# CederGroupHub/sparse-lm

Measured on AMD Instinct MI355X. Metric: fits/sec over 50-alpha Lasso path at n=100k p=5k, higher is better.
Workload: dtype f64

## Files before the change

### sparse-lm_amd/csrc/ws_kernels.hpp

```cpp
#pragma once
#include <type_traits>
#include <hip/hip_runtime.h>
#include <stdint.h>

#include "tail_kernels.hpp"
#include "newton_kernels.hpp"

namespace slm {

constexpr int WS_KCAP = 512;
constexpr int WS_KLDS = 112;
constexpr int WS_TILES = WS_KCAP / 16;
constexpr int WS_THREADS = 1024;
constexpr int WS_INNER_MAX = 400;
constexpr int WS_BB_ITERS = 14;
constexpr double WS_BB_MAX_STEP = 20.0;
constexpr double WS_INNER_TOL = 0.05;
constexpr int WS_MAX_REPEATS = 6;
constexpr int WS_NEWTON_AFTER = 16;
constexpr int WS_NEWTON_MAX = 256;
constexpr int WS_AFTER_DIRECT = 40;
constexpr double WS_NEWTON_RQ = 0.05;
constexpr int WS_NEWTON_REFUSALS = 4;
constexpr double WS_NEWTON_ENTER = 0.3;
constexpr int WS_NEWTON_RESOLVE = 5;
static_assert(NT_MAXT * NT_B == WS_KCAP, "the direct solve covers a full working set");

struct WsCtl {
  int32_t request;
  int32_t building;
  int32_t valid;
  int32_t K;
  int32_t Kreal;
  int32_t k_new;
  int32_t builds;
  int32_t appends;
  int32_t max_builds;
  int32_t disabled;
  int32_t misses;
  int32_t refined;
  int32_t counter;
  int32_t stale;
  int32_t overflows;
  int32_t sweep_new;
  int32_t sweep_miss;
  int32_t staged;
  int32_t inner_iters;
  int32_t hard;
  int32_t hard_next;
  int32_t newton_steps;
  int32_t newton_fails;
  int32_t newton_nopd;
  int32_t newton_trial[4];
  int32_t newton_ref[4];
  int32_t newton_factors;
  int32_t newton_unknowns;
  unsigned long long nt_ticks[SLM_MAX_LANES][6];
  int32_t nt_factors[SLM_MAX_LANES];
  unsigned long long solve_ticks[5];
  int32_t want_full[SLM_MAX_LANES];
  int32_t iters_hist[32];
  unsigned long long lane_ticks[SLM_MAX_LANES];
  int32_t last_point[SLM_MAX_LANES];
  int32_t repeats[SLM_MAX_LANES];
  int32_t last_cols[SLM_MAX_LANES];
  double Lw[SLM_MAX_LANES];
  int32_t carried;
  int32_t outgrown;
  int32_t served[SLM_MAX_LANES];
  int32_t hard_lane[SLM_MAX_LANES];
};

struct WsArgs {
  WsCtl* ws;
  int32_t* idx;
  int32_t* pos;
  int32_t* gs;
  int32_t* gl;
  double* score;
  double* XW;
  double* part;
  double* Gm;
  double* nt;
  double* Gx;
  const double* X;
  const double* XT;
  int64_t n, ld;
  const double* rw;
  int64_t rw_stride;
  double inv_n[SLM_MAX_LANES];
  int32_t set_of[SLM_MAX_LANES];
  int32_t set_lane[SLM_MAX_LANES];
  int32_t n_sets;
  int32_t nblk;
  const int32_t* owner;
  double theta;
  int32_t lookahead;
  int32_t append_max;
  int32_t k_init;
  int32_t bb_steps;
  int32_t one_solver;
  int32_t miss_factor;
  int32_t miss_div;
  double fill;
  int32_t power_iters;
  int32_t hard_call;
  int32_t keep_full;
};

constexpr int WS_HEAD_WORDS = 24;
static_assert(offsetof(WsCtl, hard_next) / 4 < WS_HEAD_WORDS, "the words the pass kernels decide on");
#define WS_HEAD(hd, field) ((hd)[offsetof(WsCtl, field) / 4])
__device__ __forceinline__ void ws_head_load(const WsCtl* ws, const int* gdone, int32_t* hd) {
  const int tid = threadIdx.x;
  if (tid < WS_HEAD_WORDS) hd[tid] = reinterpret_cast<const int32_t*>(ws)[tid];
  else if (tid == WS_HEAD_WORDS) hd[tid] = gdone ? gdone[0] : 0;
}

static __global__ void ws_ctl_init_kernel(WsCtl* ws, int max_builds) {
  if (threadIdx.x == 0) {
    ws->request = 1;
    ws->max_builds = max_builds;
  }
  if (threadIdx.x < SLM_MAX_LANES) ws->last_point[threadIdx.x] = -1;
}

struct BeginArgs {
  const PathCtl* h_ctl;
  PathCtl* ctl;
  const slm_path_point* h_pts;
  slm_path_point* pts;
  int64_t n_pts;
  int32_t* head;
  int32_t head_words;
  const double* lambda;
  double margin;
  double factor[SLM_MAX_LANES];
  WsCtl* ws;
  int32_t max_builds;
  int32_t n_lanes;
};
static __global__ __launch_bounds__(256) void solve_begin_kernel(SetupArgs s, BeginArgs b) {
  solve_setup_body(s);
  const int64_t stride = (int64_t)gridDim.x * blockDim.x;
  {
    static_assert(sizeof(slm_path_point) == 4 * sizeof(double), "points travel as doubles");
    const double* src = reinterpret_cast<const double*>(b.h_pts);
    double* dst = reinterpret_cast<double*>(b.pts);
    for (int64_t e = (int64_t)blockIdx.x * blockDim.x + threadIdx.x; e < 4 * b.n_pts; e += stride) dst[e] = src[e];
  }
  if (blockIdx.x != 0) return;
  for (int e = threadIdx.x; e < b.head_words; e += 256) b.head[e] = 0;
  {
    static_assert(sizeof(PathCtl) % sizeof(int32_t) == 0, "control blocks travel as words");
    const int32_t* src = reinterpret_cast<const int32_t*>(b.h_ctl);
    int32_t* dst = reinterpret_cast<int32_t*>(b.ctl);
    const int words = b.n_lanes * (int)(sizeof(PathCtl) / sizeof(int32_t));
    for (int e = threadIdx.x; e < words; e += 256) dst[e] = src[e];
  }
  __syncthreads();
  if (b.lambda != nullptr && (int)threadIdx.x < b.n_lanes && threadIdx.x < SLM_MAX_LANES) {
    const int l = threadIdx.x;
    double L0 = b.lambda[0] * b.margin;
    if (L0 <= 0.0) L0 = 1.0;
    const double L = L0 * b.factor[l];
    b.ctl[l].L = L;
    b.ctl[l].ak = 1.25 * L;
    b.ctl[l].Lhat = 0.5 * L0;
  }
  if (b.ws != nullptr) {
    if (threadIdx.x == 0) {
      b.ws->request = 1;
      b.ws->max_builds = b.max_builds;
    }
    if (threadIdx.x < SLM_MAX_LANES) b.ws->last_point[threadIdx.x] = -1;
  }
}

static __global__ __launch_bounds__(256) void ws_ctl_carry_kernel(WsCtl* ws, int max_builds) {
  __shared__ int keep_i[2];
  __shared__ double keep_L[SLM_MAX_LANES];
  if (threadIdx.x == 0) {
    keep_i[0] = ws->K;
    keep_i[1] = ws->Kreal;
  }
  if (threadIdx.x < SLM_MAX_LANES) keep_L[threadIdx.x] = ws->Lw[threadIdx.x];
  __syncthreads();
  int32_t* words = reinterpret_cast<int32_t*>(ws);
  for (int e = threadIdx.x; e < (int)(sizeof(WsCtl) / sizeof(int32_t)); e += 256) words[e] = 0;
  __syncthreads();
  if (threadIdx.x == 0) {
    ws->K = keep_i[0];
    ws->Kreal = keep_i[1];
    ws->valid = 1;
    ws->carried = 1;
    ws->max_builds = max_builds;
  }
  if (threadIdx.x < SLM_MAX_LANES) {
    ws->Lw[threadIdx.x] = keep_L[threadIdx.x];
    ws->last_point[threadIdx.x] = -1;
  }
}

__device__ __forceinline__ int block_excl_scan(int v, int* wave_tot , int* total) {
  const int lane = threadIdx.x & 63, wave = threadIdx.x >> 6;
  int inc = v;
#pragma unroll
  for (int off = 1; off < 64; off <<= 1) {
    const int t = __shfl_up(inc, off, 64);
    if (lane >= off) inc += t;
  }
  __syncthreads();
  if (lane == 63) wave_tot[wave] = inc;
  __syncthreads();
  int base = 0, tot = 0;
#pragma unroll
  for (int w = 0; w < TAIL_WAVES; ++w) {
    const int t = wave_tot[w];
    if (w < wave) base += t;
    tot += t;
  }
  *total = tot;
  return base + inc - v;
}

__device__ __forceinline__ void ws_score_body(TailArgs a, WsArgs w, const int chunk) {
  WsCtl* ws = w.ws;
  const int tid = threadIdx.x;
  __shared__ int32_t hd[WS_HEAD_WORDS + 1];
  __shared__ int lane_np[SLM_MAX_LANES];
  ws_head_load(ws, a.gdone, hd);
  if (tid < SLM_MAX_LANES) lane_np[tid] = tid < a.n_lanes ? a.ctl[tid].n_points : 0;
  __syncthreads();
  if (hd[WS_HEAD_WORDS] != 0 || WS_HEAD(hd, disabled)) return;
  const bool had_w = WS_HEAD(hd, valid) != 0;
  if (!WS_HEAD(hd, request) && !had_w) return;
  if (WS_HEAD(hd, builds) >= WS_HEAD(hd, max_builds) || WS_HEAD(hd, appends) >= 8 * WS_HEAD(hd, max_builds)) return;
  const bool singleton = a.singleton != 0;
  const int nitems = singleton ? a.p : a.G;
  __shared__ int lane_live[SLM_MAX_LANES];
  __shared__ double lane_sa[SLM_MAX_LANES], lane_sb[SLM_MAX_LANES];
  __shared__ int cnt[2];
  if (tid < SLM_MAX_LANES) {
    int live = 0;
    double sa = 0.0, sb = 0.0;
    if (tid < a.n_lanes) {
      const PathCtl* c = a.ctl + tid;
      live = !(c->done || c->idle);
      int path_end = 0;
      for (int l = 0; l < SLM_MAX_LANES; ++l) path_end = max(path_end, lane_np[l]);
      const int end = a.steal ? path_end : c->pt_off + c->n_points;
      int look = min(c->pt_off + c->point + max(w.lookahead, c->stride), end - 1);
      if (c->tail_pt >= 0 && c->point + c->stride >= c->n_points) look = c->pt_off + c->tail_pt;
      const slm_path_point pe = a.pts[look < 0 ? 0 : look];
      sa = pe.sa;
      sb = pe.sb;
    }
    lane_live[tid] = live;
    lane_sa[tid] = sa;
    lane_sb[tid] = sb;
  }
  if (tid == 0) cnt[0] = cnt[1] = 0;
  __syncthreads();

  const double inf = __builtin_huge_val();
  int n_new = 0, n_miss = 0;
  const int gt = chunk * (int)blockDim.x + tid;
  const int it = singleton ? gt : gt >> 4;
  if (singleton) {
    if (it < nitems) {
      double sc = 0.0;
      const int j = it;
      const bool in_w = had_w && w.pos[j] >= 0;
      for (int l0 = 0; l0 < a.n_lanes; l0 += 16) {
        double zp[16], zz[16], aa[16], bb[16], gg[16];
#pragma unroll
        for (int l = 0; l < 16; ++l) {
          const int ll = l0 + l < a.n_lanes ? l0 + l : 0;
          const int64_t off = (int64_t)ll * a.ld;
          zp[l] = a.zprev[off + j];
          zz[l] = a.z[off + j];
          aa[l] = a.a0[off + j];
          bb[l] = a.b0[off + j];
          gg[l] = a.g[(int64_t)ll * (a.ld + 16) + j];
        }
#pragma unroll
        for (int l = 0; l < 16; ++l) {
          if (l0 + l >= a.n_lanes || !lane_live[l0 + l]) continue;
          if (!in_w && had_w && zz[l] != zp[l]) n_miss += 1;
          if (zp[l] != 0.0) {
            sc = inf;
          } else {
            const double thr = lane_sa[l0 + l] * aa[l] + lane_sb[l0 + l] * bb[l];
            sc = fmax(sc, thr > 0.0 ? fabs(gg[l]) / thr : inf);
          }
        }
      }
      if (sc >= w.theta && !in_w) n_new += 1;
      w.score[it] = sc;
    }
  } else {
    static_assert(SLM_MAX_LANES % 16 == 0, "16-thread teams: a thread per (group, lane of a half)");
    const int l16 = tid & 15;
    const bool have = it < nitems;
    double sc = 0.0;
    bool in_w = false;
    int k0 = 0, k1 = 0;
    if (have) {
      k0 = a.gstart[it];
      k1 = a.gstart[it + 1];
      in_w = had_w && w.pos[a.order[k0]] >= 0;
    }
    for (int l = l16; have && l < a.n_lanes; l += 16) {
      if (lane_live[l]) {
        const int64_t off = (int64_t)l * a.ld;
        const double* g = a.g + (int64_t)l * (a.ld + 16);
        double num = 0.0, rmax = 0.0;
        bool act = false;
        for (int k = k0; k < k1; ++k) {
          const int j = a.order[k];
          const double zp = a.zprev[off + j], zj = a.z[off + j], aj = a.a0[off + j], gj = g[j];
          if (!in_w && had_w && zj != zp) n_miss += 1;
          act = act || zp != 0.0;
          const double thr = lane_sa[l] * aj;
          const double m = fmax(fabs(gj) - thr, 0.0);
          num = __builtin_fma(m, m, num);
          rmax = fmax(rmax, thr > 0.0 ? fabs(gj) / thr : inf);
        }
        const double den = lane_sb[l] * a.b0[off + it];
        const double r = den > 0.0 ? sqrt(num) / den : rmax;
        sc = fmax(sc, act ? inf : r);
      }
    }
#pragma unroll
    for (int o = 8; o >= 1; o >>= 1) sc = fmax(sc, __shfl_xor(sc, o, 64));
    if (have && l16 == 0) {
      if (sc >= w.theta && !in_w) n_new += k1 - k0;
      w.score[it] = sc;
    }
  }
  if (n_new) atomicAdd(&cnt[0], n_new);
  if (n_miss) atomicAdd(&cnt[1], n_miss);
  __syncthreads();
  if (tid == 0) {
    if (cnt[0]) atomicAdd(&ws->sweep_new, cnt[0]);
    if (cnt[1]) atomicAdd(&ws->sweep_miss, cnt[1]);
  }
}

static __global__ __launch_bounds__(256) void ws_score_kernel(TailArgs a, WsArgs w) { ws_score_body(a, w, (int)blockIdx.x); }

__device__ __forceinline__ void ws_select_body(TailArgs a, WsArgs w) {
  __shared__ double red[2][TAIL_WAVES];
  __shared__ int wave_tot[TAIL_WAVES];
  WsCtl* ws = w.ws;
  if (threadIdx.x < SLM_MAX_LANES) ws->served[threadIdx.x] = 0;
  if (a.gdone[0] != 0 || ws->disabled) return;
  const int tid = threadIdx.x;
  const int p = a.p, G = a.G;
  const bool singleton = a.singleton != 0;
  const int nitems = singleton ? p : G;
  const bool had_w = ws->valid != 0;

  if (tid == 0 && ws->hard_next) ws->hard = 1;
  const bool requested = ws->request != 0;
  if (!requested && !had_w) return;
  if (ws->builds >= ws->max_builds || ws->appends >= 8 * ws->max_builds) {
    if (tid == 0) {
      ws->request = 0;
      ws->stale = 1;
    }
    return;
  }

  double sweep[2] = {(double)ws->sweep_new, (double)ws->sweep_miss};
  const bool carried = ws->carried != 0;
  __syncthreads();
  if (tid == 0) {
    ws->sweep_new = 0;
    ws->sweep_miss = 0;
    ws->carried = 0;
  }
  const double inf = __builtin_huge_val();
  const bool miss = had_w && sweep[1] != 0.0;
  if (miss && tid == 0) ws->misses += 1;
  if (had_w && !requested && sweep[0] == 0.0) {
    if (miss && tid == 0) ws->stale = 1;
    return;
  }

  const int per = (nitems + WS_THREADS - 1) / WS_THREADS;
  const int i0 = tid * per, i1 = min(i0 + per, nitems);
  const bool cached = per <= 8;
  double c_sc[8];
  int c_sz[8];
  bool c_inw[8];
  if (cached) {
    int first[8];
#pragma unroll
    for (int u = 0; u < 8; ++u) {
      const int it = (i0 + u < i1) ? i0 + u : 0;
      c_sc[u] = (i0 + u < i1) ? w.score[it] : -1.0;
      first[u] = singleton ? it : a.gstart[it];
      c_sz[u] = singleton ? 1 : a.gstart[it + 1] - first[u];
    }
    if (!singleton) {
#pragma unroll
      for (int u = 0; u < 8; ++u) first[u] = a.order[first[u]];
    }
#pragma unroll
    for (int u = 0; u < 8; ++u) c_inw[u] = w.pos[first[u]] >= 0;
  }

  auto count_at = [&](double thr, bool only_new, double* n_sel, double* smax) {
    double v[2] = {0.0, 0.0};
    if (cached) {
#pragma unroll
      for (int u = 0; u < 8; ++u) {
        if (c_sc[u] >= thr && !(only_new && c_inw[u])) v[0] += (double)c_sz[u];
        if (c_sc[u] < inf) v[1] = fmax(v[1], c_sc[u]);
      }
    } else {
      for (int it = tid; it < nitems; it += WS_THREADS) {
        const double sc = w.score[it];
        const int first = singleton ? it : a.order[a.gstart[it]];
        const int size = singleton ? 1 : a.gstart[it + 1] - a.gstart[it];
        if (sc >= thr && !(only_new && w.pos[first] >= 0)) v[0] += (double)size;
        if (sc < inf) v[1] = fmax(v[1], sc);
      }
    }
    double s[1] = {v[0]};
    block_sum<1>(s, red);
    *n_sel = s[0];
    if (smax == nullptr) return;
    double m = v[1];
#pragma unroll
    for (int off = 32; off >= 1; off >>= 1) m = fmax(m, __shfl_xor(m, off, 64));
    __syncthreads();
    if ((tid & 63) == 0) red[1][tid >> 6] = m;
    __syncthreads();
    double mm = 0.0;
#pragma unroll
    for (int k = 0; k < TAIL_WAVES; ++k) mm = fmax(mm, red[1][k]);
    *smax = mm;
  };

  auto fit_threshold = [&](double thr0, bool only_new, double cap, double* n_out) -> double {
    double n_sel, smax;
    count_at(thr0, only_new, &n_sel, &smax);
    if (n_sel <= cap) {
      *n_out = n_sel;
      return thr0;
    }
    double lo = thr0, hi = fmax(smax, thr0) * (1.0 + 1e-12) + 1e-300;
    double n_hi = 0.0;
    for (int k = 0; k < 14; ++k) {
      const double mid = 0.5 * (lo + hi);
      count_at(mid, only_new, &n_sel, nullptr);
      if (n_sel > cap) {
        lo = mid;
      } else {
        hi = mid;
        n_hi = n_sel;
        if (n_sel >= w.fill * cap) break;
      }
    }
    if (n_hi == 0.0) count_at(hi, only_new, &n_hi, nullptr);
    *n_out = n_hi;
    return hi;
  };

  double n_sel, smax, thr = w.theta;
  const int k_old = had_w ? ws->Kreal : 0;
  bool append = had_w;
  if (append) {
    const int miss_mult = miss ? min(w.miss_factor, 1 + (int)sweep[1] / max(w.miss_div, 1)) : 1;
    const double cap = (double)(carried ? max(w.k_init, 4 * w.append_max) : miss_mult * w.append_max);
    if (sweep[0] <= cap) {
      n_sel = sweep[0];
    } else {
      thr = fit_threshold(w.theta, true, cap, &n_sel);
    }
    if (n_sel == 0.0) {
      if (tid == 0) ws->request = 0;
      return;
    }
    if ((double)k_old + n_sel > (double)WS_KCAP) {
      if (tid == 0) ws->outgrown += 1;
      if (w.keep_full) {
        double nz_now;
        count_at(inf, false, &nz_now, nullptr);
        if (nz_now > 0.75 * (double)WS_KCAP) {
          if (tid == 0) {
            ws->request = 0;
            ws->stale = 1;
          }
          return;
        }
      }
      append = false;
      thr = w.theta;
    }
  }
  if (!append) {
    count_at(inf, false, &n_sel, nullptr);
    if (n_sel > (double)WS_KCAP) {
      if (tid == 0) {
        ws->overflows += 1;
        ws->outgrown += 1;
        if (had_w) {
          ws->request = 0;
          ws->stale = 1;
        } else {
          ws->request = 1;
          ws->valid = 0;
          if (ws->overflows >= 50) ws->disabled = 1;
        }
      }
      return;
    }
    const double nonzeros = n_sel;
    thr = fit_threshold(w.theta, false, fmax((double)w.k_init, nonzeros), &n_sel);
    for (int j = tid; j < p; j += WS_THREADS) w.pos[j] = -1;
  }
  for (int k = k_old * (append ? 1 : 0) + tid; k < WS_KCAP; k += WS_THREADS) {
    w.idx[k] = -1;
    w.gs[k] = k;
    w.gl[k] = 1;
  }
  __syncthreads();

  unsigned long long pick = 0ull;
  int mine = 0;
  if (cached) {
#pragma unroll
    for (int u = 0; u < 8; ++u) {
      if (c_sc[u] >= thr && !(append && c_inw[u])) {
        pick |= 1ull << u;
        mine += c_sz[u];
      }
    }
  } else {
    for (int it = i0; it < i1 && it - i0 < 64; ++it) {
      if (!(w.score[it] >= thr)) continue;
      if (append && w.pos[singleton ? it : a.order[a.gstart[it]]] >= 0) continue;
      pick |= 1ull << (it - i0);
      mine += singleton ? 1 : a.gstart[it + 1] - a.gstart[it];
    }
  }
  int total = 0;
  int at = (append ? k_old : 0) + block_excl_scan(mine, wave_tot, &total);
  __syncthreads();
  for (int it = i0; it < i1 && it - i0 < 64; ++it) {
    if (!((pick >> (it - i0)) & 1ull)) continue;
    if (singleton) {
      w.idx[at] = it;
      w.pos[it] = at;
      at += 1;
    } else {
      const int k0 = a.gstart[it], len = a.gstart[it + 1] - k0;
      for (int m = 0; m < len; ++m) {
        const int j = a.order[k0 + m];
        w.idx[at + m] = j;
        w.pos[j] = at + m;
        w.gs[at + m] = at;
        w.gl[at + m] = len;
      }
      at += len;
    }
  }
  if (tid == 0) {
    const int Kreal = (append ? k_old : 0) + total;
    ws->Kreal = Kreal;
    ws->K = max(16, (Kreal + 15) & ~15);
    ws->k_new = append ? k_old : 0;
    ws->building = 1;
    ws->valid = 0;
    ws->stale = 0;
    ws->counter = 0;
    if (append) {
      ws->appends += 1;
    } else {
      ws->builds += 1;
      for (int l = 0; l < SLM_MAX_LANES; ++l) ws->Lw[l] = 0.0;
    }
  }
}

static __global__ __launch_bounds__(WS_THREADS) void ws_select_kernel(TailArgs a, WsArgs w) { ws_select_body(a, w); }

static __global__ __launch_bounds__(256) void ws_gather_kernel(WsArgs w) {
  if (!w.ws->building) return;
  const int K = w.ws->K;
  const int k0 = w.ws->k_new + 32 * (int)blockIdx.y;
  if (k0 >= K) return;
  __shared__ double tile[32][33];
  const int tx = threadIdx.x & 31, ty = threadIdx.x >> 5;
  const int64_t row_tiles = (w.n + 31) / 32;
  int jcol[4];
#pragma unroll
  for (int u = 0; u < 4; ++u) {
    const int k = k0 + ty + 8 * u;
    jcol[u] = k < K ? w.idx[k] : -1;
  }
  for (int64_t rt = blockIdx.x; rt < row_tiles; rt += gridDim.x) {
    const int64_t i0 = rt * 32;
    const int64_t i = i0 + tx;
    double v[4];
#pragma unroll
    for (int u = 0; u < 4; ++u) {
      const int j = jcol[u];
      v[u] = (j >= 0 && i < w.n) ? (w.XT ? w.XT[((rt * w.ld + j) << 5) + tx] : w.X[i * w.ld + j]) : 0.0;
    }
    __syncthreads();
#pragma unroll
    for (int u = 0; u < 4; ++u) tile[ty + 8 * u][tx] = v[u];
    __syncthreads();
    for (int ii = ty; ii < 32; ii += 8) {
      const int64_t i = i0 + ii;
      const int k = k0 + tx;
      if (i < w.n && k < K) w.XW[i * WS_KCAP + k] = tile[tx][ii];
    }
  }
}

struct XtyArgs {
  const WsCtl* ws;
  const int32_t* idx;
  const double* XW;
  const double* y;
  double* part;
  double* g;
  double* gprev;
  double* z;
  PathCtl* ctl;
  const int* done;
  int64_t n, ld;
  double inv_n;
  int n_lanes, nblk;
};
static __global__ __launch_bounds__(512) void ws_xty_partial_kernel(XtyArgs a) {
  if (*a.done) return;
  __shared__ double red[8][WS_KCAP];
  __shared__ double red_yy[8];
  const int K = a.ws->K;
  const int lane = threadIdx.x & 63, wave = threadIdx.x >> 6;
  const int64_t rows = (a.n + gridDim.x - 1) / gridDim.x;
  const int64_t i0 = (int64_t)blockIdx.x * rows, i1 = i0 + rows < a.n ? i0 + rows : a.n;
  double acc[WS_KCAP / 64];
#pragma unroll
  for (int c = 0; c < WS_KCAP / 64; ++c) acc[c] = 0.0;
  double yy = 0.0;
  auto rows4 = [&](auto NC) {
    constexpr int C = decltype(NC)::value;
    for (int64_t i = i0 + wave; i < i1; i += 32) {
      double xv[4][C], yv[4];
#pragma unroll
      for (int r = 0; r < 4; ++r) {
        const bool in = i + 8 * r < i1;
        const int64_t ii = in ? i + 8 * r : i;
        yv[r] = in ? a.y[ii] : 0.0;
#pragma unroll
        for (int c = 0; c < C; ++c) {
          const int k = lane + 64 * c;
          xv[r][c] = a.XW[ii * WS_KCAP + (k < K ? k : 64 * c)];
        }
      }
#pragma unroll
      for (int r = 0; r < 4; ++r) {
        yy = __builtin_fma(yv[r], yv[r], yy);
#pragma unroll
        for (int c = 0; c < C; ++c) acc[c] = __builtin_fma(lane + 64 * c < K ? xv[r][c] : 0.0, yv[r], acc[c]);
      }
    }
  };
  switch ((K + 63) >> 6) {
    case 1: rows4(std::integral_constant<int, 1>{}); break;
    case 2: rows4(std::integral_constant<int, 2>{}); break;
    case 3: rows4(std::integral_constant<int, 3>{}); break;
    case 4: rows4(std::integral_constant<int, 4>{}); break;
    case 5: rows4(std::integral_constant<int, 5>{}); break;
    case 6: rows4(std::integral_constant<int, 6>{}); break;
    case 7: rows4(std::integral_constant<int, 7>{}); break;
    default: rows4(std::integral_constant<int, 8>{}); break;
  }
  static_assert(WS_KCAP / 64 == 8, "eight chunks of 64 positions");
#pragma unroll
  for (int c = 0; c < WS_KCAP / 64; ++c) red[wave][lane + 64 * c] = acc[c];
  if (lane == 0) red_yy[wave] = yy;
  __syncthreads();
  double* out = a.part + (int64_t)blockIdx.x * (WS_KCAP + 1);
  const int k = threadIdx.x;
  if (k < K) {
    double sum = 0.0;
#pragma unroll
    for (int w = 0; w < 8; ++w) sum += red[w][k];
    out[k] = sum;
  }
  if (k == WS_KCAP - 1) {
    double sum = 0.0;
#pragma unroll
    for (int w = 0; w < 8; ++w) sum += red_yy[w];
    out[WS_KCAP] = sum;
  }
}
static __global__ __launch_bounds__(512) void ws_xty_apply_kernel(XtyArgs a) {
  if (*a.done) return;
  __shared__ double red[4][128];
  __shared__ double ry[512];
  const int K = a.ws->K;
  const int kl = threadIdx.x & 127, q = threadIdx.x >> 7;
  const int k = (int)blockIdx.x * 128 + kl;
  if ((int)blockIdx.x * 128 >= K) return;
  double s[8] = {0, 0, 0, 0, 0, 0, 0, 0};
  if (k < K) {
    int b = q;
    for (; b + 28 < a.nblk; b += 32) {
#pragma unroll
      for (int u = 0; u < 8; ++u) s[u] += a.part[(int64_t)(b + 4 * u) * (WS_KCAP + 1) + k];
    }
    for (; b < a.nblk; b += 4) s[0] += a.part[(int64_t)b * (WS_KCAP + 1) + k];
  }
  red[q][kl] = ((s[0] + s[1]) + (s[2] + s[3])) + ((s[4] + s[5]) + (s[6] + s[7]));
  if (blockIdx.x == 0) ry[threadIdx.x] = (int)threadIdx.x < a.nblk ? a.part[(int64_t)threadIdx.x * (WS_KCAP + 1) + WS_KCAP] : 0.0;
  __syncthreads();
  if (q == 0 && k < K) {
    const int j = a.idx[k];
    if (j >= 0) {
      const double c = -((red[0][kl] + red[1][kl]) + (red[2][kl] + red[3][kl])) * a.inv_n;
      for (int l = 0; l < a.n_lanes; ++l) {
        a.g[(int64_t)l * (a.ld + 16) + j] = c;
        a.gprev[(int64_t)l * a.ld + j] = c;
        a.z[(int64_t)l * a.ld + j] = 0.0;
      }
    }
  }
  if (blockIdx.x == 0) {
    for (int off = 256; off >= 1; off >>= 1) {
      if ((int)threadIdx.x < off) ry[threadIdx.x] += ry[threadIdx.x + off];
      __syncthreads();
    }
    if (threadIdx.x < (unsigned)a.n_lanes) {
      const int l = threadIdx.x;
      const double loss0 = 0.5 * ry[0] * a.inv_n;
      a.g[(int64_t)l * (a.ld + 16) + a.ld] = loss0;
      a.ctl[l].hist[0] = loss0;
      a.ctl[l].loss_base = loss0;
    }
  }
}

static __global__ __launch_bounds__(256) void ws_block_owner_kernel(const double* rw, int64_t rw_stride, WsArgs w, int32_t* owner) {
  __shared__ int cls[SLM_MAX_LANES];
  __shared__ int red[2][4];
  const int tid = threadIdx.x;
  const int64_t b = blockIdx.x;
  const int64_t base = w.n / w.nblk, rem = w.n % w.nblk;
  const int64_t r0 = b * base + (b < rem ? b : rem);
  const int64_t nrows = base + (b < rem ? 1 : 0);
  for (int st = 0; st < w.n_sets; ++st) {
    const double* v = rw + (int64_t)w.set_lane[st] * rw_stride + r0;
    int zeros = 1, ones = 1;
    for (int64_t i = tid; i < nrows; i += 256) {
      const double x = v[i];
      zeros &= (x == 0.0);
      ones &= (x == 1.0);
    }
    zeros = __all(zeros);
    ones = __all(ones);
    if ((tid & 63) == 0) {
      red[0][tid >> 6] = zeros;
      red[1][tid >> 6] = ones;
    }
    __syncthreads();
    if (tid == 0) {
      const int z = red[0][0] & red[0][1] & red[0][2] & red[0][3], o = red[1][0] & red[1][1] & red[1][2] & red[1][3];
      cls[st] = z ? 0 : (o ? 1 : 2);
    }
    __syncthreads();
  }
  if (tid == 0) {
    int first_ones = -1;
    for (int st = 0; st < w.n_sets; ++st) {
      int o = st;
      if (cls[st] == 0) o = -1;
      else if (cls[st] == 1) {
        if (first_ones < 0) first_ones = st;
        o = first_ones;
      }
      owner[(int64_t)st * w.nblk + b] = o;
    }
  }
}

typedef double ws_d4 __attribute__((ext_vector_type(4)));
constexpr int WS_GRAM_THREADS = 512;
constexpr int WS_GRAM_ZCHUNKS = 4;

static __global__ __launch_bounds__(WS_GRAM_THREADS) void ws_gram_kernel(WsArgs w) {
  if (!w.ws->building) return;
  __shared__ ws_d4 comb[2][16][64];
  const int K = w.ws->K;
  const int tile_lo = w.ws->k_new >> 4;
  const int tid = threadIdx.x, lane = tid & 63;
  const int wave = __builtin_amdgcn_readfirstlane(tid >> 6);
  const int tiles = K >> 4;
  const bool row_split = (tile_lo > 0 || tiles <= 8) && tiles - tile_lo <= 4 * WS_GRAM_ZCHUNKS;
  const int set = blockIdx.y;
  const int64_t b = blockIdx.x;
  if (w.owner != nullptr && w.owner[(int64_t)set * w.nblk + b] != set) return;
  const int64_t base = w.n / w.nblk, rem = w.n % w.nblk;
  const int64_t r0 = b * base + (b < rem ? b : rem);
  const int64_t nrows = base + (b < rem ? 1 : 0);
  const double* rw = w.rw ? w.rw + (int64_t)w.set_lane[set] * w.rw_stride : nullptr;
  const int part = row_split ? (wave >> 1) : 0;
  const int64_t steps = (nrows + 3) >> 2;
  const int64_t s_begin = row_split ? 4 * (steps * part / 4) : 0;
  const int64_t s_end = row_split ? min(nrows, 4 * (steps * (part + 1) / 4)) : nrows;

  for (int slice = 0; slice < 4 * WS_GRAM_ZCHUNKS; ++slice) {
  const int zhi = slice >> 2;
  if (8 * (slice & 3) >= tiles) continue;
  if (row_split ? (tile_lo + 4 * zhi >= tiles) : (zhi >= 2)) continue;
  const int wj = 2 * (slice & 3) + (wave & 1);
  const int ntj = min(4, max(0, tiles - 4 * wj));
  const int ibase = row_split ? tile_lo + 4 * zhi : 4 * (4 * zhi + (wave >> 1));
  const int ti_lo = row_split ? 0 : max(0, tile_lo - ibase);
  const int nti = min(4, max(0, tiles - ibase));
  const bool active = ti_lo < nti && ntj > 0;
  if (!row_split && !active) continue;
  ws_d4 acc[4][4];
#pragma unroll
  for (int ti = 0; ti < 4; ++ti)
#pragma unroll
    for (int tj = 0; tj < 4; ++tj) acc[ti][tj] = ws_d4{0.0, 0.0, 0.0, 0.0};

  const int kk = lane >> 4, c = lane & 15;
  if (active) {
    const int ta_max = WS_TILES - 1;
    const double* rwp = rw ? rw : w.XW;
    const bool has_rw = rw != nullptr;
    auto load = [&](int64_t s, double(&av)[4], double(&bv)[4], double& wgt) {
      const int64_t i = s + kk;
      const bool ok = i < s_end;
      const int64_t row = r0 + (ok ? i : 0);
      const double wv = rwp[has_rw ? row : 0];
      const double* xr = w.XW + row * WS_KCAP + c;
#pragma unroll
      for (int t = 0; t < 4; ++t) {
        av[t] = xr[16 * min(ibase + t, ta_max)];
        bv[t] = xr[16 * min(4 * wj + t, ta_max)];
      }
      wgt = ok ? (has_rw ? wv : 1.0) : 0.0;
    };
    auto mma = [&](const double(&av)[4], const double(&bv)[4], double wgt) {
#pragma unroll
      for (int ti = 0; ti < 4; ++ti) {
        if (ti >= ti_lo && ti < nti) {
          const double a = av[ti] * wgt;
#pragma unroll
          for (int tj = 0; tj < 4; ++tj)
            if (tj < ntj) acc[ti][tj] = __builtin_amdgcn_mfma_f64_16x16x4f64(a, bv[tj], acc[ti][tj], 0, 0, 0);
        }
      }
    };
    double a0[4], b0[4], a1[4], b1[4], a2[4], b2[4], a3[4], b3[4], w0, w1, w2, w3;
    load(s_begin, a0, b0, w0);
    load(s_begin + 4, a1, b1, w1);
    load(s_begin + 8, a2, b2, w2);
    for (int64_t s = s_begin; s < s_end; s += 16) {
      load(s + 12, a3, b3, w3);
      mma(a0, b0, w0);
      load(s + 16, a0, b0, w0);
      mma(a1, b1, w1);
      load(s + 20, a1, b1, w1);
      mma(a2, b2, w2);
      load(s + 24, a2, b2, w2);
      mma(a3, b3, w3);
    }
  }
  if (row_split) {
    for (int round = 0; round < 4; ++round) {
      if (part == round && active) {
#pragma unroll
        for (int ti = 0; ti < 4; ++ti)
#pragma unroll
          for (int tj = 0; tj < 4; ++tj) {
            if (ti < nti && tj < ntj) {
              if (round > 0) acc[ti][tj] += comb[wave & 1][ti * 4 + tj][lane];
              if (round < 3) comb[wave & 1][ti * 4 + tj][lane] = acc[ti][tj];
            }
          }
      }
      __syncthreads();
    }
  }
  if (!row_split || (part == 3 && active)) {
#pragma unroll
  for (int ti = 0; ti < 4; ++ti) {
    if (ti < ti_lo || ti >= nti) continue;
#pragma unroll
    for (int tj = 0; tj < 4; ++tj) {
      if (tj >= ntj) continue;
      const int64_t tile = (int64_t)(ibase + ti) * WS_TILES + (4 * wj + tj);
      double* out = w.part + (((int64_t)set * (WS_TILES * WS_TILES) + tile) * w.nblk + b) * 256;
#pragma unroll
      for (int r = 0; r < 4; ++r) out[(kk + 4 * r) * 16 + c] = acc[ti][tj][r];
    }
  }
  }
  if (row_split) __syncthreads();
  }
}

static __global__ __launch_bounds__(256) void ws_gram_reduce_kernel(WsArgs w) {
  WsCtl* ws = w.ws;
  if (!ws->building) return;
  const int K = ws->K;
  const int row_lo = (ws->k_new >> 4) << 4;
  const int set = blockIdx.y;
  const int tile = blockIdx.x, I = tile / WS_TILES, J = tile % WS_TILES;
  const int tiles = K >> 4, I_lo = row_lo >> 4;
  if (I < I_lo || I >= tiles || J >= tiles) return;
  const int i = 16 * I + (threadIdx.x >> 4), j = 16 * J + (threadIdx.x & 15);
  {
    const double* src = w.part + (((int64_t)set * (WS_TILES * WS_TILES) + tile) * w.nblk) * 256 + threadIdx.x;
    double s4[4] = {0.0, 0.0, 0.0, 0.0};
    int b = 0;
    if (w.owner != nullptr) {
      __shared__ int64_t off_s[512];
      static_assert(sizeof(off_s) >= 8 * 512, "nblk <= 512");
      for (int bb = threadIdx.x; bb < w.nblk; bb += 256) {
        const int o = w.owner[(int64_t)set * w.nblk + bb];
        off_s[bb] = o < 0 ? -1 : (int64_t)(o - set) * (WS_TILES * WS_TILES) * w.nblk * 256;
      }
      __syncthreads();
      for (; b + 32 <= w.nblk; b += 32) {
        double v[32];
#pragma unroll
        for (int u = 0; u < 32; ++u) {
          const int64_t o = off_s[b + u];
          v[u] = o == -1 ? 0.0 : src[(int64_t)(b + u) * 256 + o];
        }
#pragma unroll
        for (int u = 0; u < 32; ++u) s4[u & 3] += v[u];
      }
      for (; b < w.nblk; ++b) {
        const int64_t o = off_s[b];
        s4[b & 3] += o == -1 ? 0.0 : src[(int64_t)b * 256 + o];
      }
    }
    for (; b + 32 <= w.nblk; b += 32) {
      double v[32];
#pragma unroll
      for (int u = 0; u < 32; ++u) v[u] = src[(int64_t)(b + u) * 256];
#pragma unroll
      for (int u = 0; u < 32; ++u) s4[u & 3] += v[u];
    }
    for (; b < w.nblk; ++b) s4[b & 3] += src[(int64_t)b * 256];
    double s = ((s4[0] + s4[1]) + (s4[2] + s4[3])) * w.inv_n[set];
    double* Gs = (w.Gx ? w.Gx : w.Gm) + (int64_t)set * (WS_KCAP * WS_KCAP);
    Gs[i * WS_KCAP + j] = s;
    if (j < row_lo) Gs[j * WS_KCAP + i] = s;
  }
  __threadfence();
  __syncthreads();
  if (threadIdx.x == 0) {
    const int total = (tiles - I_lo) * tiles * (int)gridDim.y;
    if (atomicAdd(&ws->counter, 1) + 1 == total) {
      ws->counter = 0;
      if (w.Gx) {
        ws->staged = 1;
      } else {
        ws->request = 0;
        ws->valid = 1;
        __threadfence();
        ws->building = 0;
      }
    }
  }
}

constexpr int WS_PUBLISH_BLOCKS = 64;
static __global__ __launch_bounds__(256) void ws_publish_kernel(WsArgs w) {
  WsCtl* ws = w.ws;
  if (!ws->building || !ws->staged) return;
  const int K = ws->K;
  const int row_lo = (ws->k_new >> 4) << 4;
  const int set = blockIdx.y;
  for (int i = blockIdx.x; i < K; i += gridDim.x)
    for (int j = threadIdx.x; j < K; j += 256)
      if (i >= row_lo || j >= row_lo) {
        const int64_t at = (int64_t)set * (WS_KCAP * WS_KCAP) + (int64_t)i * WS_KCAP + j;
        w.Gm[at] = w.Gx[at];
      }
  __threadfence();
  __syncthreads();
  if (threadIdx.x == 0) {
    const int total = gridDim.x * gridDim.y;
    if (atomicAdd(&ws->counter, 1) + 1 == total) {
      ws->counter = 0;
      ws->staged = 0;
      ws->request = 0;
      ws->valid = 1;
      __threadfence();
      ws->building = 0;
    }
  }
}

constexpr int SSE_M = 16;

struct GatherArgs {
  const double* X;
  const double* XT;
  int64_t n, ld;
  const int32_t* idx;
  int K;
  double* XW;
};

static __global__ __launch_bounds__(256) void gather_cols_kernel(GatherArgs w) {
  const int k0 = 32 * (int)blockIdx.y;
  if (k0 >= w.K) return;
  __shared__ double tile[32][33];
  const int tx = threadIdx.x & 31, ty = threadIdx.x >> 5;
  const int64_t row_tiles = (w.n + 31) / 32;
  for (int64_t rt = blockIdx.x; rt < row_tiles; rt += gridDim.x) {
    const int64_t i0 = rt * 32;
    __syncthreads();
    for (int kk = ty; kk < 32; kk += 8) {
      const int k = k0 + kk;
      const int j = k < w.K ? w.idx[k] : -1;
      const int64_t i = i0 + tx;
      tile[kk][tx] = (j >= 0 && i < w.n) ? (w.XT ? w.XT[((rt * w.ld + j) << 5) + tx] : w.X[i * w.ld + j]) : 0.0;
    }
    __syncthreads();
    for (int ii = ty; ii < 32; ii += 8) {
      const int64_t i = i0 + ii;
      const int k = k0 + tx;
      if (i < w.n && k < w.K) w.XW[i * WS_KCAP + k] = tile[tx][ii];
    }
  }
}

struct SseArgs {
  const double* XW;
  const double* y;
  const double* rw;
  const double* Zs;
  double* partial;
  int64_t n;
  int K, m;
};

static __global__ __launch_bounds__(256) void sse_sparse_kernel(SseArgs a) {
  extern __shared__ double zs[];
  __shared__ double wsum[4][SSE_M];
  const int tid = threadIdx.x, lane = tid & 63, wave = tid >> 6;
  for (int e = tid; e < a.K * SSE_M; e += 256) {
    const int k = e / SSE_M, v = e - k * SSE_M;
    zs[e] = v < a.m ? a.Zs[(int64_t)v * a.K + k] : 0.0;
  }
  __syncthreads();
  double sse[SSE_M];
#pragma unroll
  for (int v = 0; v < SSE_M; ++v) sse[v] = 0.0;
  for (int64_t row = (int64_t)blockIdx.x * 256 + tid; row < a.n; row += (int64_t)gridDim.x * 256) {
    const double w = a.rw ? a.rw[row] : 1.0;
    if (w == 0.0) continue;
    const double* xr = a.XW + row * WS_KCAP;
    double dot[SSE_M];
#pragma unroll
    for (int v = 0; v < SSE_M; ++v) dot[v] = 0.0;
    for (int k = 0; k < a.K; ++k) {
      const double x = xr[k];
#pragma unroll
      for (int v = 0; v < SSE_M; ++v) dot[v] = __builtin_fma(x, zs[k * SSE_M + v], dot[v]);
    }
    const double yi = a.y[row];
#pragma unroll
    for (int v = 0; v < SSE_M; ++v) {
      const double e = dot[v] - yi;
      sse[v] = __builtin_fma(w * e, e, sse[v]);
    }
  }
#pragma unroll
  for (int v = 0; v < SSE_M; ++v) {
    double t = sse[v];
#pragma unroll
    for (int off = 32; off >= 1; off >>= 1) t += __shfl_xor(t, off, 64);
    if (lane == 0) wsum[wave][v] = t;
  }
  __syncthreads();
  if (tid < SSE_M) a.partial[(int64_t)blockIdx.x * SSE_M + tid] = wsum[0][tid] + wsum[1][tid] + wsum[2][tid] + wsum[3][tid];
}

}
```

Measured before the change: 17650.

## Compute only lower-triangle Gram tiles and template per-shape MFMA accumulation rings

Reworks the row-split path of the Gram kernel. For small fresh unweighted working sets (up to 7 tiles) it computes only the lower triangle of tiles, split across two wavefronts, and the reduce kernel mirrors the result into the upper half. Other shapes dispatch to templated rectangle kernels with exact tile counts, up to 8 column tiles per wave, and a load ring whose depth is sized to the operand count. The aim is to skip redundant symmetric MFMA work and avoid wasted clamped loads and padded accumulators. The cost is many template instantiations, which grow code size and may change register pressure.

Result: slower. 17120 (-3.0%).

```diff
diff --git a/sparse-lm_amd/csrc/ws_kernels.hpp b/sparse-lm_amd/csrc/ws_kernels.hpp
--- a/sparse-lm_amd/csrc/ws_kernels.hpp
+++ b/sparse-lm_amd/csrc/ws_kernels.hpp
@@ -1,5 +1,6 @@
 #pragma once
 #include <type_traits>
+#include <utility>
 #include <hip/hip_runtime.h>
 #include <stdint.h>
 
@@ -796,6 +797,132 @@
 typedef double ws_d4 __attribute__((ext_vector_type(4)));
 constexpr int WS_GRAM_THREADS = 512;
 constexpr int WS_GRAM_ZCHUNKS = 4;
+constexpr int WS_TRI_TILES = 7;
+
+__device__ __forceinline__ bool ws_gram_triangle(int tile_lo, int tiles, bool row_weights) {
+  return tile_lo == 0 && !row_weights && tiles <= WS_TRI_TILES;
+}
+
+template <int... Is, class F>
+__device__ __forceinline__ void ws_static_for_impl(std::integer_sequence<int, Is...>, F&& f) {
+  (f(std::integral_constant<int, Is>{}), ...);
+}
+template <int N, class F>
+__device__ __forceinline__ void ws_static_for(F&& f) {
+  ws_static_for_impl(std::make_integer_sequence<int, N>{}, f);
+}
+
+template <int T, int H>
+struct WsTri {
+  static constexpr int total = T * (T + 1) / 2;
+  static constexpr int first = H ? (total + 1) / 2 : 0;
+  static constexpr int count = H ? total - (total + 1) / 2 : (total + 1) / 2;
+  static_assert(count <= 16, "sixteen accumulator tiles per wavefront");
+  static constexpr int row(int t) {
+    int I = 0;
+    while ((I + 1) * (I + 2) / 2 <= t) ++I;
+    return I;
+  }
+  static constexpr int col(int t) { return t - row(t) * (row(t) + 1) / 2; }
+  static constexpr bool needs(int k) {
+    for (int t = first; t < first + count; ++t)
+      if (row(t) == k || col(t) == k) return true;
+    return false;
+  }
+  static constexpr int operands() {
+    int c = 0;
+    for (int k = 0; k < T; ++k) c += needs(k) ? 1 : 0;
+    return c;
+  }
+};
+
+constexpr int ws_ring_depth(int operands) {
+  const int d = 36 / (operands + 1);
+  return d < 3 ? 3 : (d > 8 ? 8 : d);
+}
+
+struct WsRows {
+  const double* xw;
+  const double* rwp;
+  bool has_rw;
+  int64_t r0, s_begin, s_end;
+  int kk;
+};
+
+template <int D, class L, class M>
+__device__ __forceinline__ void ws_gram_ring(const WsRows& R, L&& load, M&& mma) {
+  ws_static_for<D - 1>([&](auto u) { load(R.s_begin + 4 * decltype(u)::value, u); });
+  for (int64_t s = R.s_begin; s < R.s_end; s += 4 * D) {
+    ws_static_for<D>([&](auto u) {
+      constexpr int U = decltype(u)::value;
+      load(s + 4 * (U + D - 1), std::integral_constant<int, (U + D - 1) % D>{});
+      if (s + 4 * U < R.s_end) mma(u);
+    });
+  }
+}
+
+__device__ __forceinline__ const double* ws_gram_row(const WsRows& R, int64_t s, double& wgt) {
+  const int64_t i = s + R.kk;
+  const bool ok = i < R.s_end;
+  const int64_t row = R.r0 + (ok ? i : 0);
+  const double wv = R.rwp[R.has_rw ? row : 0];
+  wgt = ok ? (R.has_rw ? wv : 1.0) : 0.0;
+  return R.xw + row * WS_KCAP;
+}
+
+template <int NI, int NJ>
+__device__ __forceinline__ void ws_gram_rect(const WsRows& R, int i0, int j0, ws_d4 (&acc)[16]) {
+  static_assert(NI * NJ <= 16, "sixteen accumulator tiles per wavefront");
+  constexpr int D = ws_ring_depth(NI + NJ);
+  double xa[D][NI], xb[D][NJ], wg[D];
+  ws_gram_ring<D>(
+      R,
+      [&](int64_t s, auto st) {
+        constexpr int S = decltype(st)::value;
+        const double* xr = ws_gram_row(R, s, wg[S]);
+#pragma unroll
+        for (int t = 0; t < NI; ++t) xa[S][t] = xr[16 * (i0 + t)];
+#pragma unroll
+        for (int t = 0; t < NJ; ++t) xb[S][t] = xr[16 * (j0 + t)];
+      },
+      [&](auto st) {
+        constexpr int S = decltype(st)::value;
+#pragma unroll
+        for (int ti = 0; ti < NI; ++ti) {
+          const double a = xa[S][ti] * wg[S];
+#pragma unroll
+          for (int tj = 0; tj < NJ; ++tj)
+            acc[ti * NJ + tj] = __builtin_amdgcn_mfma_f64_16x16x4f64(a, xb[S][tj], acc[ti * NJ + tj], 0, 0, 0);
+        }
+      });
+}
+
+template <int T, int H>
+__device__ __forceinline__ void ws_gram_tri(const WsRows& R, ws_d4 (&acc)[16]) {
+  using P = WsTri<T, H>;
+  if constexpr (P::count > 0) {
+    constexpr int D = ws_ring_depth(P::operands() + 1);
+    double x[D][T], wg[D];
+    ws_gram_ring<D>(
+        R,
+        [&](int64_t s, auto st) {
+          constexpr int S = decltype(st)::value;
+          const double* xr = ws_gram_row(R, s, wg[S]);
+          ws_static_for<T>([&](auto k) {
+            constexpr int Kb = decltype(k)::value;
+            if constexpr (P::needs(Kb)) x[S][Kb] = xr[16 * Kb];
+          });
+        },
+        [&](auto st) {
+          constexpr int S = decltype(st)::value;
+          ws_static_for<P::count>([&](auto sl) {
+            constexpr int slot = decltype(sl)::value;
+            constexpr int I = P::row(P::first + slot), J = P::col(P::first + slot);
+            acc[slot] = __builtin_amdgcn_mfma_f64_16x16x4f64(x[S][I] * wg[S], x[S][J], acc[slot], 0, 0, 0);
+          });
+        });
+  }
+}
 
 static __global__ __launch_bounds__(WS_GRAM_THREADS) void ws_gram_kernel(WsArgs w) {
   if (!w.ws->building) return;
@@ -817,26 +944,113 @@
   const int64_t steps = (nrows + 3) >> 2;
   const int64_t s_begin = row_split ? 4 * (steps * part / 4) : 0;
   const int64_t s_end = row_split ? min(nrows, 4 * (steps * (part + 1) / 4)) : nrows;
-
-  for (int slice = 0; slice < 4 * WS_GRAM_ZCHUNKS; ++slice) {
+  const int kk = lane >> 4, c = lane & 15;
+  auto store_tile = [&](int I, int J, const ws_d4& t) {
+    const int64_t tile = (int64_t)I * WS_TILES + J;
+    double* out = w.part + (((int64_t)set * (WS_TILES * WS_TILES) + tile) * w.nblk + b) * 256;
+#pragma unroll
+    for (int r = 0; r < 4; ++r) out[(kk + 4 * r) * 16 + c] = t[r];
+  };
+
+  if (row_split) {
+    const int h = wave & 1;
+    const bool tri = ws_gram_triangle(tile_lo, tiles, rw != nullptr);
+    for (int ibase = tile_lo; ibase < tiles; ibase += 4) {
+      const int nti = tri ? tiles : min(4, tiles - ibase);
+      const int cap = nti <= 2 ? 8 : (nti == 3 ? 5 : 4);
+      const int sweeps = tri ? 1 : (tiles + 2 * cap - 1) / (2 * cap);
+      for (int sw = 0; sw < sweeps; ++sw) {
+        ws_d4 acc[16];
+#pragma unroll
+        for (int t = 0; t < 16; ++t) acc[t] = ws_d4{0.0, 0.0, 0.0, 0.0};
+        int sweep_zero = 0;
+        asm volatile("" : "+s"(sweep_zero));
+        const WsRows R{w.XW + c, rw ? rw : w.XW, rw != nullptr, r0, s_begin + sweep_zero, s_end, kk};
+        int cnt, j0 = 0, ntj = 0;
+        if (tri) {
+          const int total = tiles * (tiles + 1) / 2;
+          cnt = h ? total - (total + 1) / 2 : (total + 1) / 2;
+          switch (2 * tiles + h) {
+#define WS_TRI_CASE(T) \
+  case 2 * T: ws_gram_tri<T, 0>(R, acc); break; \
+  case 2 * T + 1: ws_gram_tri<T, 1>(R, acc); break;
+            WS_TRI_CASE(1) WS_TRI_CASE(2) WS_TRI_CASE(3) WS_TRI_CASE(4) WS_TRI_CASE(5) WS_TRI_CASE(6) WS_TRI_CASE(7)
+#undef WS_TRI_CASE
+            default: break;
+          }
+          static_assert(WS_TRI_TILES == 7, "an instantiation per size of the triangle");
+        } else {
+          const int c0 = tiles * sw / sweeps, c1 = tiles * (sw + 1) / sweeps;
+          const int mid = c0 + (c1 - c0 + 1) / 2;
+          j0 = h ? mid : c0;
+          ntj = h ? c1 - mid : mid - c0;
+          cnt = nti * ntj;
+          switch (8 * nti + ntj) {
+#define WS_RECT_CASE(NI, NJ) \
+  case 8 * NI + NJ: ws_gram_rect<NI, NJ>(R, ibase, j0, acc); break;
+            WS_RECT_CASE(1, 1) WS_RECT_CASE(1, 2) WS_RECT_CASE(1, 3) WS_RECT_CASE(1, 4)
+            WS_RECT_CASE(1, 5) WS_RECT_CASE(1, 6) WS_RECT_CASE(1, 7) WS_RECT_CASE(1, 8)
+            WS_RECT_CASE(2, 1) WS_RECT_CASE(2, 2) WS_RECT_CASE(2, 3) WS_RECT_CASE(2, 4)
+            WS_RECT_CASE(2, 5) WS_RECT_CASE(2, 6) WS_RECT_CASE(2, 7) WS_RECT_CASE(2, 8)
+            WS_RECT_CASE(3, 1) WS_RECT_CASE(3, 2) WS_RECT_CASE(3, 3) WS_RECT_CASE(3, 4) WS_RECT_CASE(3, 5)
+            WS_RECT_CASE(4, 1) WS_RECT_CASE(4, 2) WS_RECT_CASE(4, 3) WS_RECT_CASE(4, 4)
+#undef WS_RECT_CASE
+            default: break;
+          }
+        }
+        for (int round = 0; round < 4; ++round) {
+          if (part == round) {
+#pragma unroll
+            for (int t = 0; t < 16; ++t) {
+              if (t < cnt) {
+                if (round > 0) acc[t] += comb[h][t][lane];
+                if (round < 3) comb[h][t][lane] = acc[t];
+              }
+            }
+          }
+          __syncthreads();
+        }
+        if (part == 3) {
+          int ti = 0, tj = 0;
+          if (tri && h) {
+            const int first = (tiles * (tiles + 1) / 2 + 1) / 2;
+            while ((ti + 1) * (ti + 2) / 2 <= first) ++ti;
+            tj = first - ti * (ti + 1) / 2;
+          }
+#pragma unroll
+          for (int t = 0; t < 16; ++t) {
+            if (t < cnt) {
+              if (tri) {
+                store_tile(ti, tj, acc[t]);
+                if (++tj > ti) { ++ti; tj = 0; }
+              } else {
+                store_tile(ibase + ti, j0 + tj, acc[t]);
+                if (++tj == ntj) { ++ti; tj = 0; }
+              }
+            }
+          }
+        }
+      }
+      if (tri) break;
+    }
+    return;
+  }
+
+  for (int slice = 0; slice < 8; ++slice) {
   const int zhi = slice >> 2;
   if (8 * (slice & 3) >= tiles) continue;
-  if (row_split ? (tile_lo + 4 * zhi >= tiles) : (zhi >= 2)) continue;
   const int wj = 2 * (slice & 3) + (wave & 1);
   const int ntj = min(4, max(0, tiles - 4 * wj));
-  const int ibase = row_split ? tile_lo + 4 * zhi : 4 * (4 * zhi + (wave >> 1));
-  const int ti_lo = row_split ? 0 : max(0, tile_lo - ibase);
+  const int ibase = 4 * (4 * zhi + (wave >> 1));
+  const int ti_lo = max(0, tile_lo - ibase);
   const int nti = min(4, max(0, tiles - ibase));
-  const bool active = ti_lo < nti && ntj > 0;
-  if (!row_split && !active) continue;
+  if (ti_lo >= nti || ntj <= 0) continue;
   ws_d4 acc[4][4];
 #pragma unroll
   for (int ti = 0; ti < 4; ++ti)
 #pragma unroll
     for (int tj = 0; tj < 4; ++tj) acc[ti][tj] = ws_d4{0.0, 0.0, 0.0, 0.0};
-
-  const int kk = lane >> 4, c = lane & 15;
-  if (active) {
+  {
     const int ta_max = WS_TILES - 1;
     const double* rwp = rw ? rw : w.XW;
     const bool has_rw = rw != nullptr;
@@ -879,37 +1093,15 @@
       mma(a3, b3, w3);
     }
   }
-  if (row_split) {
-    for (int round = 0; round < 4; ++round) {
-      if (part == round && active) {
-#pragma unroll
-        for (int ti = 0; ti < 4; ++ti)
-#pragma unroll
-          for (int tj = 0; tj < 4; ++tj) {
-            if (ti < nti && tj < ntj) {
-              if (round > 0) acc[ti][tj] += comb[wave & 1][ti * 4 + tj][lane];
-              if (round < 3) comb[wave & 1][ti * 4 + tj][lane] = acc[ti][tj];
-            }
-          }
-      }
-      __syncthreads();
-    }
-  }
-  if (!row_split || (part == 3 && active)) {
 #pragma unroll
   for (int ti = 0; ti < 4; ++ti) {
     if (ti < ti_lo || ti >= nti) continue;
 #pragma unroll
     for (int tj = 0; tj < 4; ++tj) {
       if (tj >= ntj) continue;
-      const int64_t tile = (int64_t)(ibase + ti) * WS_TILES + (4 * wj + tj);
-      double* out = w.part + (((int64_t)set * (WS_TILES * WS_TILES) + tile) * w.nblk + b) * 256;
-#pragma unroll
-      for (int r = 0; r < 4; ++r) out[(kk + 4 * r) * 16 + c] = acc[ti][tj][r];
-    }
-  }
-  }
-  if (row_split) __syncthreads();
+      store_tile(ibase + ti, 4 * wj + tj, acc[ti][tj]);
+    }
+  }
   }
 }
 
@@ -921,7 +1113,8 @@
   const int set = blockIdx.y;
   const int tile = blockIdx.x, I = tile / WS_TILES, J = tile % WS_TILES;
   const int tiles = K >> 4, I_lo = row_lo >> 4;
-  if (I < I_lo || I >= tiles || J >= tiles) return;
+  const bool tri = ws_gram_triangle(I_lo, tiles, w.rw != nullptr);
+  if (I < I_lo || I >= tiles || J >= tiles || (tri && J > I)) return;
   const int i = 16 * I + (threadIdx.x >> 4), j = 16 * J + (threadIdx.x & 15);
   {
     const double* src = w.part + (((int64_t)set * (WS_TILES * WS_TILES) + tile) * w.nblk) * 256 + threadIdx.x;
@@ -961,12 +1154,12 @@
     double s = ((s4[0] + s4[1]) + (s4[2] + s4[3])) * w.inv_n[set];
     double* Gs = (w.Gx ? w.Gx : w.Gm) + (int64_t)set * (WS_KCAP * WS_KCAP);
     Gs[i * WS_KCAP + j] = s;
-    if (j < row_lo) Gs[j * WS_KCAP + i] = s;
+    if (tri ? J < I : j < row_lo) Gs[j * WS_KCAP + i] = s;
   }
   __threadfence();
   __syncthreads();
   if (threadIdx.x == 0) {
-    const int total = (tiles - I_lo) * tiles * (int)gridDim.y;
+    const int total = (tri ? tiles * (tiles + 1) / 2 : (tiles - I_lo) * tiles) * (int)gridDim.y;
     if (atomicAdd(&ws->counter, 1) + 1 == total) {
       ws->counter = 0;
       if (w.Gx) {
```
